# LucaAmbrogioni/Brancher

Hardware: AMD Instinct MI355X
Metric: ELBO iters/sec at num_samples=300 per GPU (300-sample-equivalent iterations, whole job) (higher is better)
Workload: dtype f32

## Files before the change

brancher_amd/csrc/spec_main.h:

```cpp
#pragma once

namespace bsvi {

#if defined(__HIP_DEVICE_COMPILE__)
#define SPEC_CONST_AS __attribute__((address_space(4)))
#define SPEC_GLOBAL_AS __attribute__((address_space(1)))
#define SPEC_RELOAD_ARGS() asm volatile("" : "+s"(ka))
#else
#define SPEC_CONST_AS
#define SPEC_GLOBAL_AS
#define SPEC_RELOAD_ARGS()
#endif

#define SPEC_TAB_PTR (4 * SPEC_N_UNIFORM)
#define SPEC_TAB_POS (SPEC_TAB_PTR + SPEC_N_PARAMS + 1)
#define SPEC_TAB_IDX (SPEC_TAB_POS + SPEC_N_POS)
#define SPEC_TAB_MASK (SPEC_TAB_IDX + SPEC_N_POS)

__device__ __forceinline__ void spec_lds_barrier() {
#if defined(__HIP_DEVICE_COMPILE__)
    asm volatile("s_waitcnt lgkmcnt(0)\n\ts_barrier" ::: "memory");
#endif
}

// ... 179 lines not shown
#define SPEC_VGPR_ATTR __attribute__((amdgpu_num_vgpr(SPEC_NUM_VGPR)))
#else
#define SPEC_VGPR_ATTR
#endif
#ifndef SPEC_BOUND_THREADS
#define SPEC_BOUND_THREADS SPEC_MAX_THREADS
#endif
extern "C" __global__ void __launch_bounds__(SPEC_BOUND_THREADS) SPEC_VGPR_ATTR bsvi_spec_kernel(const SpecArgs A_unused) {
    (void)A_unused;
    const SPEC_CONST_AS char* ka = (const SPEC_CONST_AS char*)__builtin_amdgcn_kernarg_segment_ptr();
#define SPEC_A ((const SPEC_CONST_AS SpecArgs*)ka)
    const uint32_t tid = threadIdx.x, nthreads = blockDim.x, W = nthreads >> 6, wave = tid >> 6, lane = tid & 63u;
    const uint32_t G = gridDim.x;
    float* const WS = spec_lds + SPEC_OFF_WS;
    float* const RED = spec_lds + SPEC_OFF_RED;
    float* const PS = spec_lds + SPEC_OFF_PS;
    uint32_t* const TAB = reinterpret_cast<uint32_t*>(spec_lds + SPEC_OFF_TAB);
    float* const WSw = WS + wave * SPEC_WS_PAD;

    SpecLane T;
    T.lane = lane;
    T.n = blockIdx.x * nthreads + tid;
    T.active = false; T.nc = 0; T.nidx = 0;
    T.vz = T.n >> 31;
    T.tile = wave * SPEC_TR_FLOATS + lane;
    const uint32_t sample_base = SPEC_A->sample_base;
    const uint32_t n_chunks = (SPEC_A->n_local + G * nthreads - 1u) / (G * nthreads);
    const uint32_t mode = SPEC_A->mode;
    const bool step = mode != SPEC_MODE_SUMS;
    const uint32_t n_it = (mode == SPEC_MODE_LOOP) ? SPEC_A->n_iterations : 1u;

#if defined(SPEC_DEBUG_STAMPS)
    const unsigned long long stamp_entry = __builtin_amdgcn_s_memtime();
#endif
    {
        const uint32_t* uniform = reinterpret_cast<const uint32_t*>(SPEC_A->uniform);
        const uint32_t* pu_ptr = SPEC_A->pu_ptr;
        const uint32_t* pu_pos = SPEC_A->pu_pos;
        const uint32_t* pu_idx = SPEC_A->pu_idx;
        const float* obs = SPEC_A->obs;
        const float* params = SPEC_A->params;
        const float* state = SPEC_A->state;
        const uint8_t* mask = SPEC_A->mask;
        const uint8_t* mask_first = SPEC_A->mask_first;
        const bool h_uni = tid < 4u * SPEC_N_UNIFORM, h_ptr = tid < SPEC_N_PARAMS + 1u, h_pos = tid < SPEC_N_POS,
                   h_obs = tid < SPEC_N_OBS, h_par = tid < SPEC_N_PARAMS;
// ... 23 lines not shown
        if (h_pos) { TAB[SPEC_TAB_POS + tid] = r_pos; TAB[SPEC_TAB_IDX + tid] = r_idx; }
        if (h_obs) spec_lds[SPEC_N_UNIFORM + tid] = r_obs;
        if (h_par) {
            PS[tid] = r_par;
            if (step) {
#pragma unroll
                for (uint32_t s = 0; s < 4u; ++s) PS[(1u + s) * SPEC_NP_PAD + tid] = r_st[s];
                TAB[SPEC_TAB_MASK + tid] = r_mask;
            }
        }
        for (uint32_t i = tid + 2u * nthreads; i < 4u * SPEC_N_UNIFORM; i += nthreads) TAB[i] = uniform[i];
        for (uint32_t i = tid + nthreads; i < SPEC_N_PARAMS + 1u; i += nthreads) TAB[SPEC_TAB_PTR + i] = pu_ptr[i];
        for (uint32_t j = tid + nthreads; j < SPEC_N_POS; j += nthreads) { TAB[SPEC_TAB_POS + j] = pu_pos[j]; TAB[SPEC_TAB_IDX + j] = pu_idx[j]; }
        for (uint32_t i = tid + nthreads; i < SPEC_N_OBS; i += nthreads) spec_lds[SPEC_N_UNIFORM + i] = obs[i];
        for (uint32_t i = tid + nthreads; i < SPEC_N_PARAMS; i += nthreads) {
            PS[i] = params[i];
            if (step) {
#pragma unroll
                for (uint32_t s = 0; s < 4u; ++s)
                    PS[(1u + s) * SPEC_NP_PAD + i] = state ? state[(size_t)s * SPEC_N_PARAMS + i] : 0.0f;
                TAB[SPEC_TAB_MASK + i] = (mask[i] ? 1u : 0u) | (mask_first[i] ? 2u : 0u);
            }
        }
        __syncthreads();
        const float* consts = SPEC_A->consts;
        for (uint32_t k = tid; k < SPEC_N_UNIFORM; k += nthreads) {
            const uint32_t src = TAB[4 * k], w1 = TAB[4 * k + 1];
            spec_publish_uniform(TAB, k, ((w1 >> 8) & 0xFFu) ? PS[src] : consts[src]);
        }
    }

    spec_f4* const OWN = reinterpret_cast<spec_f4*>(spec_lds + SPEC_OFF_OWN);
#ifndef SPEC_OWNER_WAVE
#define SPEC_OWNER_WAVE 1u
#endif
#if SPEC_TILE && SPEC_KEEP_NOISE && SPEC_KEEP_NOISE <= 68 && !SPEC_GENERIC_OWNERS && !SPEC_DIAG && !SPEC_ACCUMULATE_CHUNKS \
    && !defined(SPEC_DEBUG_NO_DRAW) && !defined(SPEC_NO_EARLY_DRAW) && !defined(SPEC_DEBUG_LATE_FREE) && defined(SPEC_WITH_DRAW_WAVE)
#define SPEC_DRAW_WAVE 1
    const uint32_t WSN = (SPEC_A->n_local + 63u) / 64u;
    const bool has_draw_wave = mode == SPEC_MODE_LOOP && G == 1u && W >= 2u && WSN < W;
    const uint32_t fed_index = W == 2u ? 0u : 1u;
    const bool draw_service = has_draw_wave && W - WSN >= 3u;
    const bool draw_wave = __builtin_amdgcn_readfirstlane((has_draw_wave && (draw_service ? wave >= WSN : wave == W - 1u)) ? 1 : 0) != 0;
    const bool fed_wave = __builtin_amdgcn_readfirstlane((has_draw_wave && (draw_service ? wave < WSN : wave == fed_index)) ? 1 : 0) != 0;
    float* const NZ = spec_lds + SPEC_OFF_TR + (draw_service ? WSN * SPEC_TR_FLOATS + wave * (SPEC_KEEP_NOISE * 64u) : (W - 1u) * SPEC_TR_FLOATS) + lane;
    float* const NZB = spec_lds + SPEC_OFF_TR + WSN * SPEC_TR_FLOATS + lane;
// ... 4 lines not shown
    const uint32_t fed_index = 1u;
#endif
#if SPEC_DRAW_WAVE && defined(SPEC_WITH_DRAW_OWNERS) && !SPEC_EXCHANGE
#define SPEC_DRAW_OWNERS 1
    const uint32_t own_wave = WSN + ((1u - WSN) & 3u);
#else
#define SPEC_DRAW_OWNERS 0
#endif
#if SPEC_DRAW_OWNERS && defined(SPEC_LEAN_CHAIN) && !defined(SPEC_DEBUG_NO_LEAN_CHAIN) && SPEC_OWN_ENTRIES == 1
#define SPEC_LEAN_OWNERS 1
#else
#define SPEC_LEAN_OWNERS 0
#endif
#if SPEC_LEAN_OWNERS && defined(SPEC_LEAN_TAIL) && !defined(SPEC_DEBUG_NO_DEFER_BOOK)
#define SPEC_DEFER_BOOK 1
#else
#define SPEC_DEFER_BOOK 0
#endif
#if SPEC_LEAN_OWNERS && defined(SPEC_LEAN_TAIL) && !defined(SPEC_DEBUG_NO_PLAIN_SGD)
#define SPEC_PLAIN_SGD 1
#else
#define SPEC_PLAIN_SGD 0
#endif
#if defined(SPEC_TAIL_MUST_BE_OFF) && (SPEC_DEFER_BOOK || SPEC_PLAIN_SGD)
#error "the tail's arrangements are compiled into a kernel that keeps the previous epilogue"
#endif
#if SPEC_DRAW_OWNERS
    const uint32_t own_base = own_wave * 64u;
#else
    const uint32_t own_base = has_draw_wave ? fed_index * 64u
                            : (!SPEC_GENERIC_OWNERS && SPEC_OWNER_WAVE * 64u + SPEC_N_PARAMS <= nthreads) ? SPEC_OWNER_WAVE * 64u : 0u;
#endif
    const uint32_t oid = tid - own_base;
    bool own_fast = false;
#if SPEC_DRAW_OWNERS
    SpecOwn own = {};
#endif
    if (oid < SPEC_N_PARAMS) {
        const uint32_t j0 = TAB[SPEC_TAB_PTR + oid], j1 = TAB[SPEC_TAB_PTR + oid + 1];
        if (j1 - j0 <= 2u) {
            own_fast = true;
#if !SPEC_DRAW_OWNERS
            SpecOwn own;
#endif
            own.n = j1 - j0;
            own.mask = 0;
            own.theta = PS[oid];
// ... 45 lines not shown
    B0.f_weight = nullptr; B0.q_weight = nullptr;
#endif
    unsigned long long off0 = ((unsigned long long)SPEC_A->offset_hi << 32) | SPEC_A->offset_lo;
    if (const unsigned long long* const offset_dev = SPEC_A->offset_dev) off0 += *offset_dev;
    const uint32_t n_global = SPEC_A->n_global;
    const uint32_t pretraining = SPEC_A->pretraining_iterations;
#if SPEC_ACCUMULATE_CHUNKS
#define SPEC_LOOP_MANY 1
#define SPEC_GEN_OVER 0x7fff0000u
    const unsigned int gen0 = 0;
    if (G > 1 && mode == SPEC_MODE_LOOP && blockIdx.x != 0 &&
        __hip_atomic_load(SPEC_A->ticket + 64, __ATOMIC_RELAXED, __HIP_MEMORY_SCOPE_AGENT) >= SPEC_GEN_OVER) return;
#else
#define SPEC_LOOP_MANY 0
#endif
#if SPEC_EXCHANGE
    uint32_t xseq0 = 0;
    if (const SpecExchange* const xg0 = SPEC_A->xchg) xseq0 = reinterpret_cast<const uint32_t*>(xg0->peer[xg0->rank])[XCHG_CALLS_WORD + 1];
#endif

#if defined(SPEC_DEBUG_STAMPS)
    unsigned long long stamp[12] = {0, 0, 0, 0, 0, 0, 0, 0, 0, 0, 0, 0};
#define SPEC_STAMP(i) if (it == n_it / 2) stamp[i] = __builtin_amdgcn_s_memtime()
    unsigned long long rstamp[7] = {0, 0, 0, 0, 0, 0, 0};
#define SPEC_RSTAMP(i) if (it == n_it / 2) rstamp[i] = __builtin_amdgcn_s_memtime()
#define SPEC_RSTAMP_NEXT() if (it == n_it / 2 + 1u) rstamp[5] = __builtin_amdgcn_s_memtime(); else if (it == 0u) stamp_first = __builtin_amdgcn_s_memtime()
    unsigned long long stamp_first = 0;
#define SPEC_RSTAMP_WRITE()                                                                                              \
    if (lane == 0u && SPEC_A->loss_slot && n_it > 16u + 8u * SPEC_MAX_WAVES) {                                           \
        asm volatile("s_waitcnt vmcnt(0)" ::: "memory");                                                                 \
        for (int i = 1; i < 7; ++i) SPEC_A->loss_slot[16u + 8u * wave + i] = rstamp[i] ? (float)(rstamp[i] - rstamp[0]) : 0.0f; \
        SPEC_A->loss_slot[16u + 8u * wave + 7] = (float)(stamp_first - stamp_entry);                                     \
        SPEC_A->loss_slot[16u + 8u * wave] = 1.0f;                                                                       \
    }
#else
#define SPEC_STAMP(i)
#define SPEC_RSTAMP(i)
#define SPEC_RSTAMP_NEXT()
#define SPEC_RSTAMP_WRITE()
#endif
#if SPEC_KEEP_NOISE && !SPEC_DIAG && !SPEC_ACCUMULATE_CHUNKS && !defined(SPEC_DEBUG_NO_DRAW) && !defined(SPEC_NO_EARLY_DRAW)
#define SPEC_EARLY_DRAW 1
    SpecNoise Z;
    bool noise_ready = false;
#else
#define SPEC_EARLY_DRAW 0
#endif
#if SPEC_DRAW_WAVE
    if (draw_service && draw_wave) {
        if (lane == 0u) { RED[8 + 2 * wave] = 0.0f; RED[9 + 2 * wave] = 0.0f; }
        const uint32_t n_draw = W - WSN, k = wave - WSN;
        const uint32_t first = k;
        uint32_t before = 0;
        for (uint32_t j = 0; j < k; ++j) before += (((WSN + j) & 3u) != 1u) ? 1u : 0u;
        const uint32_t second = n_draw + before;
        const bool has_first = first < WSN, has_second = (wave & 3u) != 1u && second < WSN;
// ... 3 lines not shown
            Tn.active = Tn.n < B0.n_local;
            Tn.nc = Tn.active ? Tn.n : (B0.n_local - 1u);
            Tn.nidx = sample_base + Tn.nc;
            Tn.off_lo = (uint32_t)offn;
            Tn.off_hi = (uint32_t)(offn >> 32);
            Tn.vz = T.vz;
            spec_draw(B0, Tn, Zd);
        };
#if SPEC_DRAW_OWNERS
        (void)has_first; (void)has_second;
        const uint32_t kown = own_wave - WSN, n_other = n_draw - 1u, rest = WSN - 1u;
        const uint32_t j = k < kown ? k : k - 1u, per = rest / n_other, extra = rest % n_other;
        const uint32_t set_a = __builtin_amdgcn_readfirstlane(1u + j * per + (j < extra ? j : extra));
        const uint32_t n_sets = __builtin_amdgcn_readfirstlane(per + (j < extra ? 1u : 0u));
        const bool owners = __builtin_amdgcn_readfirstlane(wave == own_wave ? 1 : 0) != 0;
        const float own_scale = -1.0f / (float)n_global;
        (void)own_scale;
#if SPEC_LEAN_OWNERS
        if (W != SPEC_MAX_WAVES) __builtin_trap();
#endif
#if SPEC_DEFER_BOOK
        float book_vs = 0.0f, book_finite = 0.0f;
#endif
        for (uint32_t it = 0; it < n_it; ++it) {
            const bool more = it + 1u < n_it, last = !more;
            spec_lds_barrier();
            SPEC_RSTAMP(0);
            SPEC_RSTAMP_NEXT();
            SpecNoise Za, Zb;
            float fac[2] = {0.0f, 0.0f};
            AdamBias bias = {1.0, 1.0, 0.0f, 0.0f};
            if (owners) {
                SPEC_RELOAD_ARGS();
                const bsvi_opt_cfg cfg = SPEC_A->cfg;
#pragma unroll
                for (uint32_t e = 0; e < SPEC_OWN_ENTRIES; ++e) fac[e] = own.b[e] * spec_utransform_grad(own.tr[e], own.theta);
                if (cfg.kind != BSVI_OPT_SGD) bias = optimizer_adam_bias(cfg, own.p1, own.p2);
                if (more) {
                    draw_for(0u, off0 + it + 1u, Za);
                    float* const buf = NZB + (((it + 1u) & 1u) ? WSN * (SPEC_KEEP_NOISE * 64u) : 0u);
#pragma unroll
                    for (uint32_t r = 0; r < SPEC_KEEP_NOISE; ++r) buf[64u * r] = Za.z[r];
                }
            } else if (more) {
                draw_for(set_a, off0 + it + 1u, Za);
                if (n_sets > 1u) draw_for(set_a + 1u, off0 + it + 1u, Zb);
            }
#if SPEC_LEAN_OWNERS
            typedef SPEC_GLOBAL_AS float* spec_gptr;
            spec_gptr e_out = nullptr, e_loss = nullptr, e_finite = nullptr, e_params = nullptr, e_state = nullptr;
            bsvi_opt_cfg e_cfg = {};
// ... 54 lines not shown
                    const float term = tot * fac[0];
                    gsum += own.n > 0u ? term : 0.0f;
                    grad = gsum * own_scale;
                    SPEC_RSTAMP(3);
#if SPEC_PLAIN_SGD
                    if (plain_sgd) {
                        if (finite != 0.0f && (own.mask & mask_bit)) {
                            own.st = own.st + 1.0f;
                            own.theta = own.theta - e_cfg.lr * grad;
                        }
                    } else
#endif
                    if (finite != 0.0f && (own.mask & mask_bit)) {
                        if (e_cfg.kind == BSVI_OPT_SGD) {
                            optimizer_apply(e_cfg, own.theta, own.s0, own.s1, own.s2, own.st, grad);
                        } else {
                            optimizer_apply_adam_biased(e_cfg, own.theta, own.s0, own.s1, own.s2, own.st, grad, bias);
                            own.p1 = bias.p1;
                            own.p2 = bias.p2;
                        }
                    }
                    if (more) {
                        const float g0 = utransform_common(own.tr[0], own.theta);
                        if (own.n > 0u) spec_store_uniform(own.k[0], own.a[0] + own.b[0] * g0);
                    }
                }
                asm volatile("" ::: "memory");
                SPEC_RSTAMP(6);
#if SPEC_DEFER_BOOK
                book_vs = vs; book_finite = finite;
                if (more) { SPEC_RSTAMP(4); continue; }
#endif
                const float loss = -vs / (float)n_global;
                if (oid == 0u) {
                    const float vb = spec_rows_total(rb);
                    if (last) { e_out[0] = vs; e_out[1] = vb; e_out[2] = loss; e_out[3] = finite; }
                    if (e_loss) e_loss[it] = loss;
                    if (e_finite) e_finite[it] = finite;
                }
                if (own_fast && last) {
                    e_out[BSVI_OUT_HEADER + oid] = grad;
                    e_params[oid] = own.theta;
                    if (e_state) {
                        e_state[oid] = own.s0;
                        e_state[(size_t)SPEC_N_PARAMS + oid] = own.s1;
                        e_state[2 * (size_t)SPEC_N_PARAMS + oid] = own.s2;
                        e_state[3 * (size_t)SPEC_N_PARAMS + oid] = own.st;
// ... 150 lines not shown
            spec_draw(B, T, Z);
#endif
            SPEC_STAMP(1);
            if (chunk == 0) {
                spec_lds_barrier();
                SPEC_RSTAMP(0);
                SPEC_RSTAMP_NEXT();
#if SPEC_ACCUMULATE_CHUNKS
                for (uint32_t k = lane; k < SPEC_WS_CELLS; k += 64u) WSw[k] = 0.0f;
#endif
            }
#if SPEC_DRAW_WAVE
            if (fed_wave && it > 0u) {
#if SPEC_DRAW_OWNERS
                const float* const nz = NZ + ((wave == 0u && (it & 1u)) ? WSN * (SPEC_KEEP_NOISE * 64u) : 0u);
#else
                const float* const nz = NZ;
#endif
#pragma unroll
                for (uint32_t r = 0; r < SPEC_KEEP_NOISE; ++r) Z.z[r] = nz[64u * r];
            }
#endif
            SPEC_STAMP(2);
#if !defined(SPEC_DEBUG_NO_BODY)
            if (!draw_wave) {
                spec_body(B, T, Z, WSw);
#if SPEC_TILE
                spec_du_flush(spec_lds + SPEC_OFF_TR + wave * SPEC_TR_FLOATS, WSw, lane);
#endif
            }
#endif
            SPEC_STAMP(3);
            const float value = (SPEC_ESTIMATOR == BSVI_EST_BLACKBOX) ? (T.lq * T.f + T.f) : T.f;
            lane_value += T.active ? value : 0.0f;
            lane_bad += (T.active && !isfinite(value)) ? 1.0f : 0.0f;
        }
        const float vsum = wave_sum(lane_value);
        const float bad = wave_sum(lane_bad);
        if (lane == 0) { RED[8 + 2 * wave] = vsum; RED[9 + 2 * wave] = bad; }
        SPEC_STAMP(4);
#if SPEC_EARLY_DRAW
        noise_ready = false;
#ifndef SPEC_EARLY_MASK
#define SPEC_EARLY_MASK (1u | (1u << SPEC_OWNER_WAVE))
#endif
#if defined(SPEC_DEBUG_LATE_FREE)
        if (((SPEC_EARLY_MASK >> wave) & 1u) && !((SPEC_DEBUG_LATE_FREE >> wave) & 1u) && n_chunks == 1u && it + 1u < n_it) {
#else
        if (((SPEC_EARLY_MASK >> wave) & 1u) && !has_draw_wave && n_chunks == 1u && it + 1u < n_it) {
#endif
            const unsigned long long off = off0 + it + 1u;
            SpecLane Tn = T;
            Tn.off_lo = (uint32_t)off;
            Tn.off_hi = (uint32_t)(off >> 32);
            spec_draw(B0, Tn, Z);
// ... 334 lines not shown
```

brancher_amd/csrc/spec_prelude.h:

```cpp
#pragma once
#include "bsvi_device.h"
#include "spec_args.h"

namespace bsvi {

struct SpecBody {
    const float* noise;
    float* samples_out;
    float* noise_out;
    float* fvalue_out;
    const float* f_weight;
    const float* q_weight;
    uint32_t n_local, seed_lo, seed_hi;
};

struct SpecLane {
    float f, lq;
    float gw;
    uint32_t n, nc;
    uint32_t nidx;
    uint32_t lane;
    uint32_t off_lo, off_hi;
    uint32_t vz;
    uint32_t tile;
    bool active;
};

#ifndef SPEC_KEEP_NOISE
#define SPEC_KEEP_NOISE 0
#endif
struct SpecNoise { float z[SPEC_KEEP_NOISE ? SPEC_KEEP_NOISE : 1]; };

__device__ __forceinline__ float spec_log(float x) { return __builtin_amdgcn_logf(x) * 0.6931471805599453f; }
__device__ __forceinline__ float spec_rcp(float x) { return __builtin_amdgcn_rcpf(x); }

__device__ __forceinline__ float spec_naff_lp(float v, float loc, float rS, float lS) {
    const float u = (v - loc) * rS;
    return -0.5f * (u * u) - lS - kLogSqrt2Pi;
}
__device__ __forceinline__ void spec_naff_sink(float w, float v, float loc, float rS, float lS, float& f, float& gloc, float& gS) {
    const float u = (v - loc) * rS;
    f += w * (-0.5f * (u * u) - lS - kLogSqrt2Pi);
    gloc = w * u * rS;
    gS = w * (u * u - 1.0f) * rS;
}
__device__ __forceinline__ void spec_naff_lp_bwd(float gw, float v, float loc, float rS, float& gv, float& gloc, float& gS) {
    const float d = v - loc, t = d * (rS * rS);
// ... 47 lines not shown
#define SPEC_NP_PAD ((SPEC_N_PARAMS + 3) / 4 * 4 + 4)
#define SPEC_TAB_WORDS ((4 * SPEC_N_UNIFORM + (2 * SPEC_N_PARAMS + 1) + 2 * SPEC_N_POS + 3) / 4 * 4 + 4)
#define SPEC_SCR_FLOATS (4 * (SPEC_N_POS + 2) + 4)
#define SPEC_OFF_UR SPEC_U_PAD
#define SPEC_OFF_UL (SPEC_OFF_UR + SPEC_NU_PAD)
#define SPEC_OFF_WS (SPEC_OFF_UL + SPEC_NU_PAD)
#define SPEC_OFF_RED (SPEC_OFF_WS + SPEC_MAX_WAVES * SPEC_WS_PAD)
#define SPEC_OFF_PS (SPEC_OFF_RED + SPEC_RED_FLOATS)
#define SPEC_OFF_TAB (SPEC_OFF_PS + 5 * SPEC_NP_PAD)
#define SPEC_OWN_ROWS (SPEC_N_PARAMS < SPEC_MAX_THREADS ? SPEC_N_PARAMS : SPEC_MAX_THREADS)
#define SPEC_OFF_OWN (SPEC_OFF_TAB + SPEC_TAB_WORDS)
#define SPEC_OWN_WORDS 20
#define SPEC_OFF_SCR (SPEC_OFF_OWN + SPEC_OWN_WORDS * SPEC_OWN_ROWS)
#define SPEC_OFF_TR (SPEC_OFF_SCR + SPEC_SCR_FLOATS)
#define SPEC_LDS_FLOATS (SPEC_OFF_TR + SPEC_MAX_WAVES * SPEC_TR_FLOATS)
__shared__ __attribute__((aligned(16))) float spec_lds[SPEC_LDS_FLOATS];

#define SPEC_U(k) spec_lds[(k) + T.vz]
#define SPEC_UR(k) spec_lds[SPEC_OFF_UR + (k) + T.vz]
#define SPEC_UL(k) spec_lds[SPEC_OFF_UL + (k) + T.vz]

typedef float spec_f4 __attribute__((ext_vector_type(4)));

__device__ __forceinline__ float spec_row_sum(float x) {
    x += dpp_f<0xB1>(x);
    x += dpp_f<0x4E>(x);
    x += dpp_f<0x141>(x);
    x += dpp_f<0x140>(x);
    return x;
}
#if SPEC_TILE
#define SPEC_DU(pos, val) spec_lds[SPEC_OFF_TR + T.tile + (pos) * SPEC_TR_STRIDE] = T.active ? (val) : 0.0f
__device__ __forceinline__ void spec_du_flush(const float* TRw, float* WSw, uint32_t lane) {
    asm volatile("s_waitcnt lgkmcnt(0)" ::: "memory");
    if (lane < SPEC_N_POS) {
        const spec_f4* row = reinterpret_cast<const spec_f4*>(TRw + lane * SPEC_TR_STRIDE);
        spec_f4 s = row[0];
#pragma unroll
        for (uint32_t q = 1; q < 16u; ++q) s += row[q];
        const float t = (s.x + s.y) + (s.z + s.w);
#if SPEC_ACCUMULATE_CHUNKS
        WSw[lane] += t;
#else
        WSw[lane] = t;
#endif
    }
// ... 31 lines not shown
```

brancher_amd/csrc/specialize.cpp:

```cpp
#include <hip/hip_runtime.h>
#include <hip/hiprtc.h>
#include <math.h>
#include <stdarg.h>
#include <stdio.h>
#include <stdlib.h>
#include <string.h>
#include <dlfcn.h>
#include <errno.h>
#include <fcntl.h>
#include <link.h>
#include <sys/stat.h>
#include <sys/types.h>
#include <unistd.h>

#include <algorithm>
#include <map>
#include <mutex>
#include <set>
#include <string>
#include <vector>

#include "bsvi.h"
#include "bsvi_internal.h"
#include "spec_args.h"
// ... 82 lines not shown
        for (uint32_t r : normal_rows_) s += fmt("        Z.z[%u] = A.noise[(size_t)%uu * A.n_local + T.nc];\n", r, r);
        s += "    } else {\n" + philox + "    }\n";
        return s;
    }
    const std::vector<uint32_t>& order() const { return order_; }
    std::string declarations() const {
        std::string s;
        for (uint32_t i = 0; i < d_.n_slots; ++i) s += fmt("    float v_%u = 0.0f, a_%u = 0.0f;\n", i, i);
        if (!direct_du_) for (uint32_t k = 0; k < d_.n_uniform_grad; ++k) if (du_total_[k]) s += fmt("    float du_%u = 0.0f;\n", k);
        for (uint32_t g : all_groups_) s += fmt("    float pn_%u_0 = 0.0f, pn_%u_1 = 0.0f, pn_%u_2 = 0.0f, pn_%u_3 = 0.0f;\n", g, g, g, g);
        for (uint32_t r : eps_rows_) s += fmt("    float ez_%u = 0.0f;\n", r);
        for (uint32_t r : all_node_rows_) s += fmt("    float ns_%u = 0.0f;\n", r);
        return s;
    }

private:
    const bsvi_program_desc& d_;
    bool diag_, fold_;
    bool keep_eps_ = true, counting_ = true, direct_du_ = false, reschedule_ = true, two_pass_ = false;
    int sink_mode_ = 0;
    size_t visits_ = 0;
    std::string body_;
    std::vector<uint32_t> du_total_, du_seen_, order_;
    std::set<uint32_t> sum_defined_;
    std::set<uint32_t> fwd_groups_, rev_groups_, all_groups_, eps_rows_, node_rows_, all_node_rows_, normal_rows_;

    Insn insn(uint32_t pc) const {
        Insn I;
        memcpy(&I, d_.code + 8 * (size_t)pc, 32);
        return I;
    }
    void line(const std::string& s) { if (!counting_) { body_ += "    "; body_ += s; body_ += "\n"; } }

    struct Opnd { bool lane; uint32_t idx; };
    static Opnd resolve(uint32_t o, uint32_t e) {
        const bool lane = o >> 31;
        const uint32_t step = ((o >> 30) & 1u) * (lane ? 8u : 4u);
        const uint32_t off = (o & 0x3FFFFFFFu) + e * step;
        return Opnd{lane, lane ? off / 8u : off / 4u};
    }
    std::string val(uint32_t o, uint32_t e) const {
        const Opnd p = resolve(o, e);
        return p.lane ? fmt("v_%u", p.idx) : fmt("SPEC_U(%u)", p.idx);
    }
    int literal(uint32_t o, uint32_t e) const {
        if (!fold_) return -1;
// ... 67 lines not shown
        eps_rows_.insert(row);
        line(fmt("ez_%u = noise ? noise[(size_t)%uu * A.n_local + T.nc] : %s;", row, row, pn.c_str()));
        return fmt("ez_%u", row);
    }
    std::string eps_reverse(uint32_t row) {
        if (keep_eps_) return fmt("Z.z[%u]", row);
        const std::string pn = normal_var(row, true);
        if (!diag_) return pn;
        line(fmt("ez_%u = noise ? noise[(size_t)%uu * A.n_local + T.nc] : %s;", row, row, pn.c_str()));
        return fmt("ez_%u", row);
    }
    void diag_outputs(uint32_t row, const std::string& v, const std::string& noise) {
        if (!diag_) return;
        line(fmt("if (T.active) { if (A.samples_out) A.samples_out[(size_t)%uu * A.n_local + T.n] = %s; "
                 "if (A.noise_out) A.noise_out[(size_t)%uu * A.n_local + T.n] = %s; }", row, v.c_str(), row, noise.c_str()));
    }

    void forward(const Insn& I, uint32_t e, bool nodes) {
        const uint32_t op = I.w0 & 0xFFu, flags = (I.w0 >> 8) & 0xFFu, dist = (I.w0 >> 16) & 0xFFu;
        if (op == BSVI_OP_NAFF) {
            if (!nodes) return;
            ++visits_;
            if (counting_) return;
            line("{");
            line(fmt("  const float loc = %s;", affine(I.a, I.b, I.c, e).c_str()));
            std::string v = val(I.dst, e);
            if (flags & BSVI_F_SAMPLE) {
                const uint32_t row = resolve(I.dst, e).idx;
                const std::string eps = eps_forward(row);
                if (flags & BSVI_F_GIVEN) line(fmt("  %s = %s;", v.c_str(), eps.c_str()));
                else { line(fmt("  %s = loc + %s * %s;", v.c_str(), eps.c_str(), val(I.s, e).c_str())); sum_defined_.insert(row); }
                diag_outputs(row, v, eps);
            }
            if (flags & (BSVI_F_ENT | BSVI_F_LOGP | BSVI_F_WF)) line(fmt("  const float lS = %s;", log_of(I.s, e).c_str()));
            if (flags & BSVI_F_ENT) line(fmt("  %s += %s * (kHalfLog2PiE + lS);", ftarget(), flit(I.imm1).c_str()));
            if (flags & (BSVI_F_LOGP | BSVI_F_WF)) {
                line(fmt("  const float lp = spec_naff_lp(%s, loc, %s, lS);", v.c_str(), rcp_of(I.s, e).c_str()));
                line(fmt("  %s += %s * lp;", ftarget(), flit(I.imm0).c_str()));
                if ((flags & BSVI_F_WF) && sink_mode_ != 2) line("  T.lq += lp;");
            }
            line("}");
        } else if (op == BSVI_OP_BIN) {
            ++visits_;
            if (counting_) return;
            const std::string a = val(I.a, e), b = val(I.b, e), y = val(I.dst, e);
            switch (flags) {
            case BSVI_B_ADD: line(fmt("%s = %s + %s;", y.c_str(), a.c_str(), b.c_str())); break;
            case BSVI_B_SUB: line(fmt("%s = %s - %s;", y.c_str(), a.c_str(), b.c_str())); break;
            case BSVI_B_MUL: line(fmt("%s = %s * %s;", y.c_str(), a.c_str(), b.c_str())); break;
            case BSVI_B_DIV: line(fmt("%s = %s / %s;", y.c_str(), a.c_str(), b.c_str())); break;
            case BSVI_B_POW: line(fmt("%s = pow_ff(%s, %s);", y.c_str(), a.c_str(), b.c_str())); break;
            default: line(fmt("%s = (%s == %s) ? 1.0f : 0.0f;", y.c_str(), a.c_str(), b.c_str())); break;
            }
        } else if (op == BSVI_OP_UN) {
            ++visits_;
            if (counting_) return;
            line(fmt("%s = unop<true>(%uu, %s, %s);", val(I.dst, e).c_str(), flags, val(I.a, e).c_str(), flit(I.imm0).c_str()));
        } else if (op == BSVI_OP_NODE) {
            if (!nodes) return;
            ++visits_;
            if (counting_) return;
            line("{");
            line(fmt("  const float p0 = %s, p1 = %s;", val(I.a, e).c_str(), val(I.b, e).c_str()));
            const std::string v = val(I.dst, e);
            if (flags & BSVI_F_SAMPLE) {
                const uint32_t row = resolve(I.dst, e).idx;
                node_rows_.insert(row);
                all_node_rows_.insert(row);
                const std::string draw = fmt("{ const float2 dr = philox_draw(spec_key(A, T), %u, p0, p1, %uu); %s = dr.x; ns_%u = dr.y; }",
                                             dist, row, v.c_str(), row);
                if (diag_) {
                    const std::string given = (flags & BSVI_F_GIVEN) ? fmt("ns_%u", row) : fmt("sample_from_noise_generic(%u, p0, p1, ns_%u)", dist, row);
                    line(fmt("  if (noise) { ns_%u = noise[(size_t)%uu * A.n_local + T.nc]; %s = %s; } else %s", row, row, v.c_str(), given.c_str(), draw.c_str()));
                } else {
                    line("  " + draw);
                }
                diag_outputs(row, v, fmt("ns_%u", row));
            }
            if (flags & BSVI_F_ENT) line(fmt("  %s += %s * entropy_generic(%u, p0, p1);", ftarget(), flit(I.imm1).c_str(), dist));
            if (flags & (BSVI_F_LOGP | BSVI_F_WF)) {
                line(fmt("  const float lp = logp_generic(%u, %s, p0, p1);", dist, v.c_str()));
                line(fmt("  %s += %s * lp;", ftarget(), flit(I.imm0).c_str()));
                if ((flags & BSVI_F_WF) && sink_mode_ != 2) line("  T.lq += lp;");
            }
            line("}");
        }
    }

    const char* ftarget() const { return sink_mode_ == 2 ? "f_dead" : "T.f"; }

    std::string wg(uint32_t imm) const { return diag_ ? "(" + flit(imm) + " * T.gw)" : flit(imm); }

    void naff_sink(const Insn& I, uint32_t e) {
        ++visits_;
        const std::string loc = affine(I.a, I.b, I.c, e);
        if (sink_mode_ == 1) {
            line(fmt("T.f += %s * spec_naff_lp(%s, %s, %s, %s);", flit(I.imm0).c_str(), val(I.dst, e).c_str(), loc.c_str(),
                     rcp_of(I.s, e).c_str(), log_of(I.s, e).c_str()));
            return;
        }
        if (!counting_) {
            line("{");
            line(fmt("  float gl, gs; spec_naff_sink(%s, %s, %s, %s, %s, %s, gl, gs);", flit(I.imm0).c_str(), val(I.dst, e).c_str(),
                     loc.c_str(), rcp_of(I.s, e).c_str(), log_of(I.s, e).c_str(), ftarget()));
            if (diag_) line("  gl *= T.gw; gs *= T.gw;");
        }
        add_adj(I.dst, e, "-gl");
        add_adj_times(I.a, e, "gl", I.b);
        add_adj_times(I.b, e, "gl", I.a);
        add_adj(I.c, e, "gl");
        add_adj(I.s, e, "gs");
        line("}");
    }

    void backward(const Insn& I, uint32_t e) {
        const uint32_t op = I.w0 & 0xFFu, flags = (I.w0 >> 8) & 0xFFu, dist = (I.w0 >> 16) & 0xFFu;
        ++visits_;
// ... 123 lines not shown
            for (uint32_t j = 0; j < R.n; ++j) forward(insn(R.first + j), e, false);
            zero_temps(R.temp_base, R.n_temps);
            for (uint32_t j = R.n; j-- > 0;) backward(insn(R.first + j), e);
        }
    }
    void slots_of(const Item& R, std::set<uint32_t>& reads, std::set<uint32_t>& writes) const {
        for (uint32_t j = 0; j < R.n; ++j) {
            const Insn I = insn(R.first + j);
            const uint32_t op = I.w0 & 0xFFu, flags = (I.w0 >> 8) & 0xFFu;
            const uint32_t ops[5] = {I.dst, I.a, I.b, I.c, I.s};
            const int n_opnd = (op == BSVI_OP_NAFF) ? 5 : ((op == BSVI_OP_UN) ? 2 : 3);
            const bool defines = op == BSVI_OP_BIN || op == BSVI_OP_UN || (flags & BSVI_F_SAMPLE);
            for (uint32_t e = 0; e < R.n_elems; ++e)
                for (int k = 0; k < n_opnd; ++k) {
                    const Opnd p = resolve(ops[k], e);
                    if (!p.lane) continue;
                    if (k == 0 && defines) writes.insert(p.idx); else reads.insert(p.idx);
                }
        }
    }

    void walk() {
        visits_ = 0;
        const std::vector<Item> recs = items();
        std::vector<std::pair<int, int>> key(recs.size(), std::make_pair(-1, -1));
        std::vector<int> def_of(d_.n_slots, -1);
        std::vector<uint32_t> rorder;
        for (uint32_t r = 0; r < recs.size(); ++r) {
            if (recs[r].sink) continue;
            std::set<uint32_t> rd, wr;
            slots_of(recs[r], rd, wr);
            bool samples = false;
            for (uint32_t j = 0; j < recs[r].n; ++j) {
                const Insn I = insn(recs[r].first + j);
                const uint32_t op = I.w0 & 0xFFu;
                if ((op == BSVI_OP_NAFF || op == BSVI_OP_NODE) && (((I.w0 >> 8) & 0xFFu) & BSVI_F_SAMPLE)) samples = true;
            }
            int anchor = (int)r;
            if (!samples && reschedule_) {
                int a = -1;
                for (uint32_t sl : rd) {
                    if (sl >= recs[r].temp_base && sl < recs[r].temp_base + recs[r].n_temps) continue;
                    if (def_of[sl] >= 0 && key[def_of[sl]].first > a) a = key[def_of[sl]].first;
                }
                if (a >= 0) anchor = a;
            }
// ... 10 lines not shown
                std::set<uint32_t> rd, wr;
                slots_of(recs[r], rd, wr);
                int first = -1;
                for (uint32_t sl : rd) {
                    if (sl >= recs[r].temp_base && sl < recs[r].temp_base + recs[r].n_temps) continue;
                    const int dr = def_of[sl];
                    if (dr >= 0 && (uint32_t)dr < r && (first < 0 || key[dr] > key[first])) first = dr;
                }
                if (first >= 0) { home[r] = first; deferred[first].push_back(r); }
            }
        }
        const bool fence = d_.n_code > kFenceAboveCode;
        uint32_t since = 0;
        auto maybe_fence = [&]() { if (fence && ++since >= kFenceEvery) { since = 0; line("asm volatile(\"\" ::: \"memory\"); __builtin_amdgcn_sched_barrier(0);"); } };
        if (two_pass_) line("float f_dead = 0.0f; (void)f_dead;");
        for (uint32_t r = 0; r < recs.size(); ++r) {
            if (home[r] >= 0 && !two_pass_) continue;
            sink_mode_ = home[r] >= 0 ? 1 : 0;
            emit_forward(recs[r]);
            sink_mode_ = 0;
            maybe_fence();
            if (visits_ > kMaxVisits) return;
        }
        if (diag_) line("const float fweight = A.q_weight ? A.q_weight[T.nc] : T.f * T.gw; (void)fweight;");
        else line("const float fweight = T.f; (void)fweight;");
        if (fence) {
            line("asm volatile(\"\" ::: \"memory\");");
            for (uint32_t s0 = 0; s0 < d_.n_slots; s0 += 16) {
                std::string ops;
                for (uint32_t sl = s0; sl < d_.n_slots && sl < s0 + 16; ++sl) ops += fmt("%s\"+v\"(v_%u)", sl == s0 ? "" : ", ", sl);
                line("asm volatile(\"\" : " + ops + ");");
            }
        }
        for (uint32_t r : rorder) {
            sink_mode_ = two_pass_ ? 2 : 0;
            for (uint32_t sidx : deferred[r]) emit_forward(recs[sidx]);
            sink_mode_ = 0;
            emit_reverse(recs[r]);
            maybe_fence();
            if (visits_ > kMaxVisits) return;
        }
        if (diag_) line("if (A.fvalue_out && T.active) { A.fvalue_out[T.n] = T.f; A.fvalue_out[(size_t)A.n_local + T.n] = T.lq; }");
    }
};

}
// ... 66 lines not shown
    const uint32_t live = 2 * d.n_slots + (d.n_noise <= kKeepEpsRows ? d.n_noise : 0) + (d.n_uniform_grad <= kAccumulateEntries ? d.n_uniform_grad : 0) + 40;
    auto fit = [&](uint32_t threads, Geom& g) {
        g.max_threads = threads;
        g.lds_bytes = lds_floats(d.n_params, d.n_uniform, d.n_obs, s->n_pos, threads, (int)(&g - s->geom)) * 4u;
        return g.lds_bytes <= 160u * 1024u;
    };
    bool ok = (live <= 232 && fit(512, s->geom[GEOM_ONE])) || fit(256, s->geom[GEOM_ONE]);
    ok = ok && fit(256, s->geom[GEOM_MANY]);
    if (!ok) { why = "the program's tables do not fit LDS"; delete s; return nullptr; }
    bool all_fast = d.n_params <= 64;
    for (uint32_t i = 0; i < d.n_params && all_fast; ++i) all_fast = s->pu_ptr_host[i + 1] - s->pu_ptr_host[i] <= 2;
    s->draw_wave_ok = all_fast && tiled(s->n_pos, GEOM_ONE) && d.n_noise > 0 && d.n_noise <= kKeepEpsRows;
    uint32_t ut_mask = 0;
    for (uint32_t k = 0; k < d.n_uniform; ++k) ut_mask |= 1u << (d.uniform[k].transform & 31u);
    const bool rare_transforms = (ut_mask >> (BSVI_UT_SIGMOID + 1)) != 0;
    uint32_t own_entries = 1;
    for (uint32_t i = 0; i < d.n_params; ++i) own_entries = std::max(own_entries, std::min(2u, s->pu_ptr_host[i + 1] - s->pu_ptr_host[i]));
    const char* const lean_env = getenv("BSVI_SPEC_LEAN_BODY");
    const bool lean_body = !(lean_env && lean_env[0] == '0');
    const bool want_previous = getenv("BSVI_SPEC_LEAN_CHAIN") != nullptr;
    std::string previous;
    const char* const tail_env = getenv("BSVI_SPEC_TAIL");
    const bool tail = !(tail_env && tail_env[0] == '0');
    for (int gi = 0; gi < 2; ++gi) {
        const Geom& G = s->geom[gi];
        for (int v = 0; v < (gi == GEOM_ONE && want_previous ? 3 : 2); ++v) {
            const bool old = v == 2;
            const bool lean = lean_body && !old;
            Emitter E(d, v == 1, lean);
            if (!E.run(why)) { delete s; return nullptr; }
            std::string src;
            src += "// generated by libbsvi (specialize.cpp) from a model program: do not edit\n";
            src += "#define BSVI_SPECIALIZED 1\n";
            const char* const slp = getenv("BSVI_JIT_SLP");
            if (slp ? slp[0] == '0' : (d.n_code > kFenceAboveCode && d.estimator == BSVI_EST_BLACKBOX))
                src += std::string(kJitOptionMark) + "-fno-slp-vectorize\n";
            const char* const ra = getenv("BSVI_JIT_REGALLOC");
            if (ra ? ra[0] == 'b' : d.n_code > kBasicRegallocAboveCode)
                src += std::string(kJitOptionMark) + "-mllvm\n" + kJitOptionMark + "-vgpr-regalloc=basic\n";
            src += fmt("#define SPEC_N_PARAMS %u\n#define SPEC_N_UNIFORM %u\n#define SPEC_N_UGRAD %u\n#define SPEC_N_OBS %u\n#define SPEC_N_NOISE %u\n",
                       d.n_params, d.n_uniform, d.n_uniform_grad, d.n_obs, d.n_noise);
            src += fmt("#define SPEC_N_POS %u\n", s->n_pos);
            src += fmt("#define SPEC_ESTIMATOR %u\n#define SPEC_MAX_THREADS %u\n#define SPEC_DIAG %d\n", d.estimator, G.max_threads, v == 1 ? 1 : 0);
            src += fmt("#define SPEC_ACCUMULATE_CHUNKS %d\n#define SPEC_TILE %d\n", gi == GEOM_MANY ? 1 : 0, tiled(s->n_pos, gi) ? 1 : 0);
            if (gi == GEOM_MANY && many_waves() > 2) src += fmt("#define SPEC_BOUND_THREADS %u\n", 256u * many_waves());
            src += fmt("#define SPEC_KEEP_NOISE %u\n", E.keeps_noise() ? d.n_noise : 0u);
            src += fmt("#define SPEC_GENERIC_OWNERS %d\n", all_fast ? 0 : 1);
            src += fmt("#define SPEC_RARE_TRANSFORMS %d\n#define SPEC_UT_MASK 0x%xu\n", rare_transforms ? 1 : 0, ut_mask);
            if (!old) src += fmt("#define SPEC_OWN_ENTRIES %u\n", own_entries);
            src += "#include \"spec_prelude.h\"\n";
            src += "namespace bsvi {\n";
            src += "__device__ __forceinline__ void spec_draw(const SpecBody& A, const SpecLane& T, SpecNoise& Z) {\n";
            src += "    (void)A; (void)T; (void)Z;\n";
            src += E.draw();
            src += "}\n";
            src += "__device__ __forceinline__ void spec_body(const SpecBody& A, SpecLane& T, const SpecNoise& Z, float* WSw) {\n";
            src += "    (void)Z;\n";
            if (v == 1) src += "    const float* const noise = A.noise;\n";
            if (old) { previous = std::move(src); previous += E.declarations() + E.body() + "}\n}  // namespace bsvi\n#include \"spec_main.h\"\n"; continue; }
            src += E.declarations();
            src += E.body();
            src += "}\n}  // namespace bsvi\n";
            src += "#include \"spec_main.h\"\n";
            s->variant[2 * gi + v].src = std::move(src);
        }
    }
    s->variant[4].src = "#define SPEC_WITH_DRAW_WAVE 1\n" + s->variant[0].src;
    s->variant[6].src = std::string("#define SPEC_WITH_DRAW_WAVE 1\n#define SPEC_WITH_DRAW_OWNERS 1\n#define SPEC_LEAN_CHAIN 1\n")
                        + (tail ? "#define SPEC_LEAN_TAIL 1\n" : "") + s->variant[0].src;
    if (want_previous) s->variant[7].src = "#define SPEC_WITH_DRAW_WAVE 1\n#define SPEC_WITH_DRAW_OWNERS 1\n" + previous;
    s->exchange_ok = true;
    s->variant[5].src = std::string("#define SPEC_WITH_EXCHANGE 1\n") + (s->draw_wave_ok ? "#define SPEC_WITH_DRAW_WAVE 1\n" : "") + s->variant[0].src;
    return s;
}

void destroy(Spec* s) {
    if (!s) return;
    for (Variant& v : s->variant) if (v.module) (void)hipModuleUnload(v.module);
    if (s->dev) (void)hipFree(s->dev);
    delete s;
}

int upload(Spec* s) {
    const size_t n_ptr = s->pu_ptr_host.size(), n_pos = s->pu_pos_host.size();
    const size_t bytes = 512 + (n_ptr + 2 * n_pos) * 4 + 256;
    hipError_t e = hipMalloc(&s->dev, bytes);
    if (e != hipSuccess) return bsvi_fail(BSVI_ERR_HIP, std::string("hipMalloc (specialiser tables): ") + hipGetErrorString(e));
    std::vector<uint32_t> host(128 + n_ptr + 2 * n_pos, 0u);
    std::copy(s->pu_ptr_host.begin(), s->pu_ptr_host.end(), host.begin() + 128);
    std::copy(s->pu_pos_host.begin(), s->pu_pos_host.end(), host.begin() + 128 + n_ptr);
    std::copy(s->pu_idx_host.begin(), s->pu_idx_host.end(), host.begin() + 128 + n_ptr + n_pos);
    e = hipMemset(s->dev, 0, bytes);
// ... 379 lines not shown
```

Measured before the change: 303,700.

## Stage uniform table publish so body overlaps owners' reciprocal/log computation

```diff
diff --git a/brancher_amd/csrc/spec_main.h b/brancher_amd/csrc/spec_main.h
--- a/brancher_amd/csrc/spec_main.h
+++ b/brancher_amd/csrc/spec_main.h
@@ -225,6 +225,10 @@
     T.lane = lane;
     T.n = blockIdx.x * nthreads + tid;
     T.active = false; T.nc = 0; T.nidx = 0;
+    T.it = 0; T.ready = 0; T.late = 0;
+#if defined(SPEC_DEBUG_STAMPS)
+    T.t_ready = 0; T.polls = 0;
+#endif
     T.vz = T.n >> 31;
     T.tile = wave * SPEC_TR_FLOATS + lane;
     const uint32_t sample_base = SPEC_A->sample_base;
@@ -294,6 +298,7 @@
                 TAB[SPEC_TAB_MASK + i] = (mask[i] ? 1u : 0u) | (mask_first[i] ? 2u : 0u);
             }
         }
+        if (tid == 0u) reinterpret_cast<uint32_t*>(spec_lds)[SPEC_OFF_READY] = 0u;
         __syncthreads();
         const float* consts = SPEC_A->consts;
         for (uint32_t k = tid; k < SPEC_N_UNIFORM; k += nthreads) {
@@ -344,7 +349,10 @@
 #else
 #define SPEC_PLAIN_SGD 0
 #endif
-#if defined(SPEC_TAIL_MUST_BE_OFF) && (SPEC_DEFER_BOOK || SPEC_PLAIN_SGD)
+#if SPEC_STAGED && !(SPEC_LEAN_OWNERS && defined(SPEC_LEAN_TAIL))
+#error "the body waits for a ready word that these owners do not write"
+#endif
+#if defined(SPEC_TAIL_MUST_BE_OFF) && (SPEC_DEFER_BOOK || SPEC_PLAIN_SGD || SPEC_STAGED)
 #error "the tail's arrangements are compiled into a kernel that keeps the previous epilogue"
 #endif
 #if SPEC_DRAW_OWNERS
@@ -436,16 +444,16 @@
 #if defined(SPEC_DEBUG_STAMPS)
     unsigned long long stamp[12] = {0, 0, 0, 0, 0, 0, 0, 0, 0, 0, 0, 0};
 #define SPEC_STAMP(i) if (it == n_it / 2) stamp[i] = __builtin_amdgcn_s_memtime()
-    unsigned long long rstamp[7] = {0, 0, 0, 0, 0, 0, 0};
+    unsigned long long rstamp[10] = {0, 0, 0, 0, 0, 0, 0, 0, 0, 0};
 #define SPEC_RSTAMP(i) if (it == n_it / 2) rstamp[i] = __builtin_amdgcn_s_memtime()
 #define SPEC_RSTAMP_NEXT() if (it == n_it / 2 + 1u) rstamp[5] = __builtin_amdgcn_s_memtime(); else if (it == 0u) stamp_first = __builtin_amdgcn_s_memtime()
     unsigned long long stamp_first = 0;
 #define SPEC_RSTAMP_WRITE()                                                                                              \
-    if (lane == 0u && SPEC_A->loss_slot && n_it > 16u + 8u * SPEC_MAX_WAVES) {                                           \
+    if (lane == 0u && SPEC_A->loss_slot && n_it > 16u + 16u * SPEC_MAX_WAVES) {                                          \
         asm volatile("s_waitcnt vmcnt(0)" ::: "memory");                                                                 \
-        for (int i = 1; i < 7; ++i) SPEC_A->loss_slot[16u + 8u * wave + i] = rstamp[i] ? (float)(rstamp[i] - rstamp[0]) : 0.0f; \
-        SPEC_A->loss_slot[16u + 8u * wave + 7] = (float)(stamp_first - stamp_entry);                                     \
-        SPEC_A->loss_slot[16u + 8u * wave] = 1.0f;                                                                       \
+        for (int i = 1; i < 10; ++i) if (i != 7) SPEC_A->loss_slot[16u + 16u * wave + i] = rstamp[i] ? (float)(rstamp[i] - rstamp[0]) : 0.0f; \
+        SPEC_A->loss_slot[16u + 16u * wave + 7] = (float)(stamp_first - stamp_entry);                                    \
+        SPEC_A->loss_slot[16u + 16u * wave] = 1.0f;                                                                      \
     }
 #else
 #define SPEC_STAMP(i)
@@ -495,11 +503,27 @@
 #if SPEC_DEFER_BOOK
         float book_vs = 0.0f, book_finite = 0.0f;
 #endif
+#if SPEC_STAGED
+        float staged_u = 1.0f;
+#endif
         for (uint32_t it = 0; it < n_it; ++it) {
             const bool more = it + 1u < n_it, last = !more;
             spec_lds_barrier();
             SPEC_RSTAMP(0);
             SPEC_RSTAMP_NEXT();
+#if SPEC_STAGED
+            if (owners && it > 0u) {
+                if (own_fast && own.n > 0u) {
+                    spec_lds[SPEC_OFF_UR + own.k[0]] = spec_rcp(staged_u);
+                    spec_lds[SPEC_OFF_UL + own.k[0]] = spec_log(staged_u);
+                }
+#if defined(__HIP_DEVICE_COMPILE__)
+                asm volatile("s_waitcnt lgkmcnt(0)" ::: "memory");
+#endif
+                if (lane == 0u) reinterpret_cast<uint32_t*>(spec_lds)[SPEC_OFF_READY] = it;
+                SPEC_RSTAMP(8);
+            }
+#endif
             SpecNoise Za, Zb;
             float fac[2] = {0.0f, 0.0f};
             AdamBias bias = {1.0, 1.0, 0.0f, 0.0f};
@@ -600,7 +624,12 @@
                     }
                     if (more) {
                         const float g0 = utransform_common(own.tr[0], own.theta);
+#if SPEC_STAGED
+                        staged_u = own.a[0] + own.b[0] * g0;
+                        if (own.n > 0u) spec_lds[own.k[0]] = staged_u;
+#else
                         if (own.n > 0u) spec_store_uniform(own.k[0], own.a[0] + own.b[0] * g0);
+#endif
                     }
                 }
                 asm volatile("" ::: "memory");
@@ -797,15 +826,31 @@
             }
 #endif
             SPEC_STAMP(2);
+#if SPEC_STAGED
+            T.it = it;
+            T.ready = reinterpret_cast<const uint32_t*>(spec_lds)[SPEC_OFF_READY + T.vz];
+#endif
 #if !defined(SPEC_DEBUG_NO_BODY)
             if (!draw_wave) {
+#if defined(SPEC_DEBUG_BODY_PRIO)
+                if (wave == 4u) __builtin_amdgcn_s_setprio(SPEC_DEBUG_BODY_PRIO);
+#endif
                 spec_body(B, T, Z, WSw);
 #if SPEC_TILE
                 spec_du_flush(spec_lds + SPEC_OFF_TR + wave * SPEC_TR_FLOATS, WSw, lane);
 #endif
+#if defined(SPEC_DEBUG_BODY_PRIO)
+                if (wave == 4u) __builtin_amdgcn_s_setprio(0);
+#endif
             }
 #endif
             SPEC_STAMP(3);
+#if SPEC_STAGED
+            if (T.late != 0u) T.f = __int_as_float(0x7fc00000);
+#if defined(SPEC_DEBUG_STAMPS)
+            if (it == n_it / 2) { rstamp[8] = T.t_ready; rstamp[9] = rstamp[0] + T.polls; }
+#endif
+#endif
             const float value = (SPEC_ESTIMATOR == BSVI_EST_BLACKBOX) ? (T.lq * T.f + T.f) : T.f;
             lane_value += T.active ? value : 0.0f;
             lane_bad += (T.active && !isfinite(value)) ? 1.0f : 0.0f;
diff --git a/brancher_amd/csrc/spec_prelude.h b/brancher_amd/csrc/spec_prelude.h
--- a/brancher_amd/csrc/spec_prelude.h
+++ b/brancher_amd/csrc/spec_prelude.h
@@ -23,6 +23,12 @@
     uint32_t off_lo, off_hi;
     uint32_t vz;
     uint32_t tile;
+    uint32_t it, ready;
+    uint32_t late;
+#if defined(SPEC_DEBUG_STAMPS)
+    unsigned long long t_ready;
+    uint32_t polls;
+#endif
     bool active;
 };
 
@@ -116,6 +122,59 @@
 
 typedef float spec_f4 __attribute__((ext_vector_type(4)));
 
+#if defined(SPEC_LEAN_TAIL) && defined(SPEC_LEAN_CHAIN) && defined(SPEC_WITH_DRAW_OWNERS) && defined(SPEC_WITH_DRAW_WAVE)          \
+    && !defined(SPEC_WITH_EXCHANGE) && SPEC_TILE && SPEC_KEEP_NOISE && SPEC_KEEP_NOISE <= 68 && !SPEC_GENERIC_OWNERS && !SPEC_DIAG \
+    && !SPEC_ACCUMULATE_CHUNKS && !defined(SPEC_DEBUG_NO_DRAW) && !defined(SPEC_NO_EARLY_DRAW) && !defined(SPEC_DEBUG_LATE_FREE) \
+    && !defined(SPEC_DEBUG_NO_LEAN_CHAIN) && defined(SPEC_OWN_ENTRIES) && SPEC_OWN_ENTRIES == 1                                  \
+    && !defined(SPEC_STAGED_OFF) && !defined(SPEC_DEBUG_NO_STAGED_PUBLISH)
+#define SPEC_STAGED 1
+#else
+#define SPEC_STAGED 0
+#endif
+#define SPEC_OFF_READY (SPEC_OFF_RED + 4)
+#ifndef SPEC_READY_POLLS
+#define SPEC_READY_POLLS 65536u
+#endif
+#define SPEC_ENT_NOW(f, w, k) { const float lS_ = SPEC_UL(k); f += (w) * (kHalfLog2PiE + lS_); }
+#if SPEC_STAGED
+__device__ __forceinline__ void spec_table_ready(SpecLane& T, float& swept) {
+#if defined(__HIP_DEVICE_COMPILE__)
+    asm volatile("" : "+v"(swept));
+#endif
+#if defined(SPEC_DEBUG_STAMPS)
+    T.t_ready = __builtin_amdgcn_s_memtime();
+#endif
+    uint32_t word = __builtin_amdgcn_readfirstlane(T.ready);
+    if (word != T.it && T.late == 0u) {
+#if defined(__HIP_DEVICE_COMPILE__)
+        typedef const volatile __attribute__((address_space(3))) uint32_t* spec_ready_ptr;
+#else
+        typedef const volatile uint32_t* spec_ready_ptr;
+#endif
+        const spec_ready_ptr ready = (spec_ready_ptr)(spec_lds + SPEC_OFF_READY);
+        uint32_t polls = 0;
+        do {
+            __builtin_amdgcn_s_sleep(1);
+            word = __builtin_amdgcn_readfirstlane(ready[T.vz]);
+        } while (word != T.it && ++polls < SPEC_READY_POLLS);
+        if (word != T.it) T.late = 1u;
+#if defined(SPEC_DEBUG_STAMPS)
+        T.polls = polls + 1u;
+#endif
+    }
+#if defined(__HIP_DEVICE_COMPILE__)
+    asm volatile("" ::: "memory");
+#endif
+}
+#define SPEC_ENT_FWD(f, w, k)
+#define SPEC_ENT_LATE(f, w, k) SPEC_ENT_NOW(f, w, k)
+#define SPEC_TABLE_READY(swept) spec_table_ready(T, swept)
+#else
+#define SPEC_ENT_FWD(f, w, k) SPEC_ENT_NOW(f, w, k)
+#define SPEC_ENT_LATE(f, w, k)
+#define SPEC_TABLE_READY(swept)
+#endif
+
 __device__ __forceinline__ float spec_row_sum(float x) {
     x += dpp_f<0xB1>(x);
     x += dpp_f<0x4E>(x);
diff --git a/brancher_amd/csrc/specialize.cpp b/brancher_amd/csrc/specialize.cpp
--- a/brancher_amd/csrc/specialize.cpp
+++ b/brancher_amd/csrc/specialize.cpp
@@ -128,6 +128,9 @@
     size_t visits_ = 0;
     std::string body_;
     std::vector<uint32_t> du_total_, du_seen_, order_;
+    bool table_ready_ = false;
+    std::vector<std::string> late_ent_;
+    std::string swept_;
     std::set<uint32_t> sum_defined_;
     std::set<uint32_t> fwd_groups_, rev_groups_, all_groups_, eps_rows_, node_rows_, all_node_rows_, normal_rows_;
 
@@ -241,6 +244,9 @@
             if (!nodes) return;
             ++visits_;
             if (counting_) return;
+            const bool term = (flags & (BSVI_F_ENT | BSVI_F_LOGP | BSVI_F_WF)) != 0;
+            const bool ent_hook = !table_ready_ && (flags & (BSVI_F_ENT | BSVI_F_LOGP | BSVI_F_WF)) == BSVI_F_ENT && !resolve(I.s, e).lane;
+            if (term && !ent_hook) table_ready();
             line("{");
             line(fmt("  const float loc = %s;", affine(I.a, I.b, I.c, e).c_str()));
             std::string v = val(I.dst, e);
@@ -251,7 +257,15 @@
                 else { line(fmt("  %s = loc + %s * %s;", v.c_str(), eps.c_str(), val(I.s, e).c_str())); sum_defined_.insert(row); }
                 diag_outputs(row, v, eps);
             }
-            if (flags & (BSVI_F_ENT | BSVI_F_LOGP | BSVI_F_WF)) line(fmt("  const float lS = %s;", log_of(I.s, e).c_str()));
+            if (ent_hook) {
+                const std::string args = fmt("%s, %s, %uu", ftarget(), flit(I.imm1).c_str(), resolve(I.s, e).idx);
+                line("  SPEC_ENT_FWD(" + args + ");");
+                late_ent_.push_back(args);
+                swept_ = v;
+                line("}");
+                return;
+            }
+            if (term) line(fmt("  const float lS = %s;", log_of(I.s, e).c_str()));
             if (flags & BSVI_F_ENT) line(fmt("  %s += %s * (kHalfLog2PiE + lS);", ftarget(), flit(I.imm1).c_str()));
             if (flags & (BSVI_F_LOGP | BSVI_F_WF)) {
                 line(fmt("  const float lp = spec_naff_lp(%s, loc, %s, lS);", v.c_str(), rcp_of(I.s, e).c_str()));
@@ -279,6 +293,7 @@
             if (!nodes) return;
             ++visits_;
             if (counting_) return;
+            table_ready();
             line("{");
             line(fmt("  const float p0 = %s, p1 = %s;", val(I.a, e).c_str(), val(I.b, e).c_str()));
             const std::string v = val(I.dst, e);
@@ -306,12 +321,20 @@
         }
     }
 
+    void table_ready() {
+        if (table_ready_) return;
+        table_ready_ = true;
+        line("SPEC_TABLE_READY(" + swept_ + ");");
+        for (const std::string& args : late_ent_) line("SPEC_ENT_LATE(" + args + ");");
+    }
+
     const char* ftarget() const { return sink_mode_ == 2 ? "f_dead" : "T.f"; }
 
     std::string wg(uint32_t imm) const { return diag_ ? "(" + flit(imm) + " * T.gw)" : flit(imm); }
 
     void naff_sink(const Insn& I, uint32_t e) {
         ++visits_;
+        table_ready();
         const std::string loc = affine(I.a, I.b, I.c, e);
         if (sink_mode_ == 1) {
             line(fmt("T.f += %s * spec_naff_lp(%s, %s, %s, %s);", flit(I.imm0).c_str(), val(I.dst, e).c_str(), loc.c_str(),
@@ -481,6 +504,9 @@
 
     void walk() {
         visits_ = 0;
+        table_ready_ = false;
+        late_ent_.clear();
+        swept_ = "T.f";
         const std::vector<Item> recs = items();
         std::vector<std::pair<int, int>> key(recs.size(), std::make_pair(-1, -1));
         std::vector<int> def_of(d_.n_slots, -1);
@@ -537,6 +563,7 @@
             maybe_fence();
             if (visits_ > kMaxVisits) return;
         }
+        table_ready();
         if (diag_) line("const float fweight = A.q_weight ? A.q_weight[T.nc] : T.f * T.gw; (void)fweight;");
         else line("const float fweight = T.f; (void)fweight;");
         if (fence) {
@@ -649,6 +676,8 @@
     std::string previous;
     const char* const tail_env = getenv("BSVI_SPEC_TAIL");
     const bool tail = !(tail_env && tail_env[0] == '0');
+    const char* const staged_env = getenv("BSVI_SPEC_STAGED");
+    const bool staged = !(staged_env && staged_env[0] == '0');
     for (int gi = 0; gi < 2; ++gi) {
         const Geom& G = s->geom[gi];
         for (int v = 0; v < (gi == GEOM_ONE && want_previous ? 3 : 2); ++v) {
@@ -694,7 +723,7 @@
     }
     s->variant[4].src = "#define SPEC_WITH_DRAW_WAVE 1\n" + s->variant[0].src;
     s->variant[6].src = std::string("#define SPEC_WITH_DRAW_WAVE 1\n#define SPEC_WITH_DRAW_OWNERS 1\n#define SPEC_LEAN_CHAIN 1\n")
-                        + (tail ? "#define SPEC_LEAN_TAIL 1\n" : "") + s->variant[0].src;
+                        + (tail ? "#define SPEC_LEAN_TAIL 1\n" : "") + (staged ? "" : "#define SPEC_STAGED_OFF 1\n") + s->variant[0].src;
     if (want_previous) s->variant[7].src = "#define SPEC_WITH_DRAW_WAVE 1\n#define SPEC_WITH_DRAW_OWNERS 1\n" + previous;
     s->exchange_ok = true;
     s->variant[5].src = std::string("#define SPEC_WITH_EXCHANGE 1\n") + (s->draw_wave_ok ? "#define SPEC_WITH_DRAW_WAVE 1\n" : "") + s->variant[0].src;
```

After: 300,800. About the same (-1.0%).
